# XuyangBai/D3Feat

Measured on AMD Instinct MI355X. Metric: fragments/sec (30k-pt clouds), higher is better.
Workload: dtype f32; 1 GPU; SURVEY §8d config #2: synthetic 3DMatch room fragment, 300k raw pts -> grid subsample 0.03 m (~29k pts per cloud) -> self-pair -> 5-level pyramid -> full KPFCNN forward (random-init weights (reference initialiser, seed 42), 14.1M params)...; points_per_cloud=29369, fragments_per_gpu=2141, parallelism=fragment-dp1, fragments_per_replay=12, engine_fallbacks=0, engine_isolated_replays=0

## Files before the change

### d3feat_amd/csrc/pool_head.hip

```cpp
#include "common.h"

template <int VEC, class FT = float, bool U24 = false>
__global__ void __launch_bounds__(256) maxpool_kernel(const FT* __restrict__ x, int N1, int ldx, int C,
                                                      const int* __restrict__ idx, int N2, int ld_idx, int K,
                                                      FT* __restrict__ out, int ldo,
                                                      const int* __restrict__ N1_dev, const int* __restrict__ N2_dev,
                                                      const int* __restrict__ row_order) {
    N1 = d3f_dyn(N1, N1_dev);
    N2 = d3f_dyn(N2, N2_dev);
    const int CV = C / VEC;
    const unsigned nblk = (unsigned)(((long long)N2 * CV + 255) / 256);
    if (blockIdx.x >= nblk) return;
    const long long t = (long long)d3f_xcd_tile(blockIdx.x, nblk) * 256 + threadIdx.x;
    if (t >= (long long)N2 * CV) return;
    int slot, c;
    if (U24) { const unsigned tu = (unsigned)t; slot = (int)(tu / (unsigned)CV); c = (int)(tu - (unsigned)slot * (unsigned)CV) * VEC; }
    else { slot = (int)(t / CV); c = (int)(t % CV) * VEC; }
    const int n = row_order ? row_order[slot] : slot;
    float m[VEC];
#pragma unroll
    for (int v = 0; v < VEC; ++v) m[v] = -3.402823466e38f;
    const int* row = U24 ? idx + __umul24((unsigned)n, (unsigned)ld_idx) : idx + (size_t)n * ld_idx;
    int nvalid = 0;
    constexpr int NB = 8;
    for (int k0 = 0; k0 < K; k0 += NB) {
        int id[NB];
        float val[NB][VEC];
#pragma unroll
        for (int j = 0; j < NB; ++j) id[j] = (k0 + j < K) ? row[k0 + j] : -2;
#pragma unroll
        for (int j = 0; j < NB; ++j) {
            const bool ok = id[j] >= 0 && id[j] < N1;
            nvalid += ok ? 1 : 0;
            if (ok) {
                const FT* xr = U24 ? x + (__umul24((unsigned)id[j], (unsigned)ldx) + (unsigned)c) : x + ((size_t)id[j] * ldx + c);
                if (VEC == 4) {
                    const float4 f = D3fFeat<FT>::ld4(xr);
                    val[j][0] = f.x; val[j][1 % VEC] = f.y; val[j][2 % VEC] = f.z; val[j][3 % VEC] = f.w;
                } else {
#pragma unroll
                    for (int v = 0; v < VEC; ++v) val[j][v] = D3fFeat<FT>::ld1(xr + v);
                }
            } else {
#pragma unroll
                for (int v = 0; v < VEC; ++v) val[j][v] = -3.402823466e38f;
            }
        }
#pragma unroll
        for (int j = 0; j < NB; ++j)
#pragma unroll
            for (int v = 0; v < VEC; ++v) m[v] = fmaxf(m[v], val[j][v]);
    }
    if (nvalid == 0) {
        unsigned om[VEC];
#pragma unroll
        for (int v = 0; v < VEC; ++v) om[v] = 0xFFFFFFFFu;
        for (int r0 = 0; r0 < N1; r0 += 4) {
            float val[4][VEC];
#pragma unroll
            for (int j = 0; j < 4; ++j) {
                const int r = min(r0 + j, N1 - 1);
                const FT* xr = x + ((size_t)r * ldx + c);
                if (VEC == 4) {
                    const float4 f = D3fFeat<FT>::ld4(xr);
                    val[j][0] = f.x; val[j][1 % VEC] = f.y; val[j][2 % VEC] = f.z; val[j][3 % VEC] = f.w;
                } else {
#pragma unroll
                    for (int v = 0; v < VEC; ++v) val[j][v] = D3fFeat<FT>::ld1(xr + v);
                }
            }
#pragma unroll
            for (int j = 0; j < 4; ++j)
#pragma unroll
                for (int v = 0; v < VEC; ++v) om[v] = min(om[v], d3f_f2ord(val[j][v]));
        }
#pragma unroll
        for (int v = 0; v < VEC; ++v) m[v] = d3f_ord2f(om[v]);
    }
#pragma unroll
    for (int v = 0; v < VEC; ++v) D3fFeat<FT>::st1(&out[(size_t)n * ldo + c + v], m[v]);
}

extern "C" int d3f_ind_max_pool(const void* x_, int N1, int ldx, int C, const int* idx, int N2, int ld_idx, int K,
                                void* out_, int ldo, float* col_min_dev, const int* N1_dev, const int* N2_dev,
                                const int* row_order, int feat_bf16, void* stream_) {
    hipStream_t stream = (hipStream_t)stream_;
    const float* x = (const float*)x_;
    float* out = (float*)out_;
    (void)col_min_dev;
    if (N1 < 0 || N2 < 0 || C < 1 || ldx < C || ldo < C || K < 0 || ld_idx < K) return D3F_ERR_ARG;
    if (N2 == 0) return D3F_OK;
    if (!x || !idx || !out) return D3F_ERR_ARG;
    const bool u24 = d3f_fits_u24(N1, ldx) && d3f_fits_u24(N2, ld_idx) && (long long)N2 * C < (1ll << 31);
    if (feat_bf16) {
        if (C % 4 || ldx % 4 || ((uintptr_t)x_ & 7)) return D3F_ERR_ARG;
        const unsigned short* xh = (const unsigned short*)x_;
        unsigned short* oh = (unsigned short*)out_;
        if (u24)
            maxpool_kernel<4, unsigned short, true><<<d3f_cdiv((long long)N2 * (C / 4), 256), 256, 0, stream>>>(
                xh, N1, ldx, C, idx, N2, ld_idx, K, oh, ldo, N1_dev, N2_dev, row_order);
        else
            maxpool_kernel<4, unsigned short><<<d3f_cdiv((long long)N2 * (C / 4), 256), 256, 0, stream>>>(
                xh, N1, ldx, C, idx, N2, ld_idx, K, oh, ldo, N1_dev, N2_dev, row_order);
        D3F_LAUNCH_CHECK();
        return D3F_OK;
    }
    if (C % 4 == 0 && ldx % 4 == 0 && (((uintptr_t)x) & 15) == 0 && u24)
        maxpool_kernel<4, float, true><<<d3f_cdiv((long long)N2 * (C / 4), 256), 256, 0, stream>>>(x, N1, ldx, C, idx, N2, ld_idx, K,
                                                                                                   out, ldo, N1_dev, N2_dev, row_order);
    else if (C % 4 == 0 && ldx % 4 == 0 && (((uintptr_t)x) & 15) == 0)
        maxpool_kernel<4><<<d3f_cdiv((long long)N2 * (C / 4), 256), 256, 0, stream>>>(x, N1, ldx, C, idx, N2, ld_idx, K,
                                                                                      out, ldo, N1_dev, N2_dev, row_order);
    else
        maxpool_kernel<1><<<d3f_cdiv((long long)N2 * C, 256), 256, 0, stream>>>(x, N1, ldx, C, idx, N2, ld_idx, K,
                                                                               out, ldo, N1_dev, N2_dev, row_order);
    D3F_LAUNCH_CHECK();
    return D3F_OK;
}

__global__ void __launch_bounds__(256) upsample_cat_kernel(const float* __restrict__ x, int N1, int ldx, int C1,
                                                           const int* __restrict__ idx, int N2, int ld_idx,
                                                           const float* __restrict__ skip, int lds, int C2,
                                                           float* __restrict__ out, int ldo, const int* __restrict__ N1_dev,
                                                           const int* __restrict__ N2_dev) {
    N1 = d3f_dyn(N1, N1_dev);
    N2 = d3f_dyn(N2, N2_dev);
    const int Ct = C1 + C2;
    const long long t = (long long)blockIdx.x * blockDim.x + threadIdx.x;
    if (t >= (long long)N2 * Ct) return;
    const int n = (int)(t / Ct), c = (int)(t % Ct);
    float v;
    if (c < C1) {
        const int id = idx[(size_t)n * ld_idx];
        v = (id >= 0 && id < N1) ? x[(size_t)id * ldx + c] : 0.f;
    } else {
        v = skip[(size_t)n * lds + (c - C1)];
    }
    out[(size_t)n * ldo + c] = v;
}

extern "C" int d3f_closest_pool_cat(const float* x, int N1, int ldx, int C1, const int* idx, int N2, int ld_idx,
                                    const float* skip, int lds, int C2, float* out, int ldo, const int* N1_dev,
                                    const int* N2_dev, void* stream_) {
    hipStream_t stream = (hipStream_t)stream_;
    if (N1 < 0 || N2 < 0 || C1 < 1 || C2 < 0 || ldx < C1 || ldo < C1 + C2 || ld_idx < 1 || (C2 > 0 && lds < C2))
        return D3F_ERR_ARG;
    if (N2 == 0) return D3F_OK;
    if (!x || !idx || !out || (C2 > 0 && !skip)) return D3F_ERR_ARG;
    upsample_cat_kernel<<<d3f_cdiv((long long)N2 * (C1 + C2), 256), 256, 0, stream>>>(x, N1, ldx, C1, idx, N2, ld_idx, skip,
                                                                                      lds, C2, out, ldo, N1_dev, N2_dev);
    D3F_LAUNCH_CHECK();
    return D3F_OK;
}

__global__ void __launch_bounds__(256) head_max_init_kernel(const int* __restrict__ lens, const int* __restrict__ include_zero_dev,
                                                            int group, int B, unsigned* __restrict__ mx, int* __restrict__ offs) {
    __shared__ int slen[256];
    const int b = threadIdx.x;
    const int len = b < B ? lens[b] : 0;
    const int inc_in = (include_zero_dev && b < B) ? include_zero_dev[b] : 0;
    slen[b] = len;
    __syncthreads();
    if (b >= B) return;
    const int g = group > 0 ? group : B;
    const int g0 = b / g * g, g1 = min(g0 + g, B);
    int before = 0;
    for (int j = 0; j < b; ++j) before += slen[j];
    int longest = 0, all_eq = 1;
    for (int j = g0; j < g1; ++j) longest = max(longest, slen[j]);
    for (int j = g0; j < g1; ++j) all_eq &= (slen[j] == longest);
    offs[b] = before;
    const int inc = include_zero_dev ? inc_in : ((len < longest || all_eq) ? 1 : 0);
    mx[b] = inc ? d3f_f2ord(0.f) : 0u;
    if (b == B - 1) offs[B] = before + len;
}

template <bool DENSE>
__global__ void __launch_bounds__(256) head_max_kernel(const float* __restrict__ x, int N, int ldx, int C,
                                                       const int* __restrict__ offs, int B, unsigned* __restrict__ mx) {
    const int b = blockIdx.y;
    const long long lo = (long long)offs[b] * C, hi = (long long)offs[b + 1] * C;
    unsigned m = 0u;
    if (DENSE) {
        const long long lo4 = lo >> 2, hi4 = hi >> 2;
        const long long stride = (long long)gridDim.x * blockDim.x;
        long long t = lo4 + (long long)blockIdx.x * blockDim.x + threadIdx.x;
        for (; t + 3 * stride < hi4; t += 4 * stride) {
            float4 v[4];
#pragma unroll
            for (int u = 0; u < 4; ++u) v[u] = ((const float4*)x)[t + u * stride];
#pragma unroll
            for (int u = 0; u < 4; ++u)
                m = max(max(m, d3f_f2ord(v[u].x)), max(d3f_f2ord(v[u].y), max(d3f_f2ord(v[u].z), d3f_f2ord(v[u].w))));
        }
        for (; t < hi4; t += stride) {
            const float4 v = ((const float4*)x)[t];
            m = max(max(m, d3f_f2ord(v.x)), max(d3f_f2ord(v.y), max(d3f_f2ord(v.z), d3f_f2ord(v.w))));
        }
    } else {
        for (long long t = lo + (long long)blockIdx.x * blockDim.x + threadIdx.x; t < hi; t += (long long)gridDim.x * blockDim.x) {
            const long long r = t / C;
            const int c = (int)(t % C);
            m = max(m, d3f_f2ord(x[(size_t)r * ldx + c]));
        }
    }
#pragma unroll
    for (int o = 32; o > 0; o >>= 1) m = max(m, (unsigned)__shfl_xor((int)m, o, 64));
    __shared__ unsigned red[4];
    if ((threadIdx.x & 63) == 0) red[threadIdx.x >> 6] = m;
    __syncthreads();
    if (threadIdx.x == 0 && lo < hi) atomicMax(&mx[b], max(max(red[0], red[1]), max(red[2], red[3])));
}

template <int CPL>
__global__ void __launch_bounds__(256)
head_kernel(const float* __restrict__ x, int N, int ldx, int C, const int* __restrict__ idx, int ld_idx, int K,
            const int* __restrict__ offs, int B, const unsigned* __restrict__ mx, float* __restrict__ desc, int ldd,
            float* __restrict__ score, const int* __restrict__ row_order) {
    N = min(N, offs[B]);
    if ((int)(blockIdx.x * 8) >= N) return;
    const int half = (int)d3f_xcd_tile(blockIdx.x, (unsigned)((N + 7) / 8)) * 8 + (threadIdx.x >> 5), l = threadIdx.x & 31;
    const bool active = half < N;
    const int n = active ? (row_order ? row_order[half] : half) : 0;
    const int b = d3f_find_elem(offs, B, n);
    const float den = d3f_ord2f(mx[b]) + 1e-6f;
    float xv[CPL], yv[CPL], sum[CPL];
    float sq = 0.f;
#pragma unroll
    for (int j = 0; j < CPL; ++j) {
        const int c = l + 32 * j;
        xv[j] = (c < C) ? x[(size_t)n * ldx + c] : 0.f;
        yv[j] = xv[j] / den;
        sum[j] = 0.f;
        sq += xv[j] * xv[j];
    }
#pragma unroll
    for (int o = 16; o > 0; o >>= 1) sq += __shfl_xor(sq, o, 64);
    int cnt = 0;
    const int hbase = threadIdx.x & 32;
    for (int k0 = 0; k0 < K; k0 += 32) {
        const int mine = (k0 + l < K) ? idx[(size_t)n * ld_idx + k0 + l] : -1;
        const int kn = min(32, K - k0);
        for (int kk = 0; kk < kn; kk += 4) {
            int id[4];
            float dn[4];
            float v[4][CPL];
#pragma unroll
            for (int j = 0; j < 4; ++j) {
                id[j] = __shfl(mine, hbase + min(kk + j, 31), 64);
                if (kk + j >= kn || id[j] < 0 || id[j] >= N) id[j] = -1;
            }
#pragma unroll
            for (int j = 0; j < 4; ++j) {
                dn[j] = 1.f;
                if (id[j] >= 0) dn[j] = d3f_ord2f(mx[d3f_find_elem(offs, B, id[j])]) + 1e-6f;
#pragma unroll
                for (int jj = 0; jj < CPL; ++jj) {
                    const int c = l + 32 * jj;
                    v[j][jj] = (id[j] >= 0 && c < C) ? x[(size_t)id[j] * ldx + c] : 0.f;
                }
            }
#pragma unroll
            for (int j = 0; j < 4; ++j) {
                float rs = 0.f;
#pragma unroll
                for (int jj = 0; jj < CPL; ++jj) {
                    const float y = v[j][jj] / dn[j];
                    sum[jj] += y;
                    rs += y;
                }
#pragma unroll
                for (int o = 16; o > 0; o >>= 1) rs += __shfl_xor(rs, o, 64);
                cnt += (id[j] >= 0 && rs != 0.f) ? 1 : 0;
            }
        }
    }
    const float fc = (float)max(cnt, 1);
    float ymax = -3.402823466e38f;
#pragma unroll
    for (int j = 0; j < CPL; ++j)
        if (l + 32 * j < C) ymax = fmaxf(ymax, yv[j]);
#pragma unroll
    for (int o = 16; o > 0; o >>= 1) ymax = fmaxf(ymax, __shfl_xor(ymax, o, 64));
    float best = -3.402823466e38f;
#pragma unroll
    for (int j = 0; j < CPL; ++j) {
        if (l + 32 * j < C) {
            const float d = yv[j] - sum[j] / fc;
            float sp;
            if (d > 15.f) sp = d;
            else if (d < -15.f) sp = expf(d);
            else sp = log1pf(expf(d));
            best = fmaxf(best, sp * (yv[j] / (1e-6f + ymax)));
        }
    }
#pragma unroll
    for (int o = 16; o > 0; o >>= 1) best = fmaxf(best, __shfl_xor(best, o, 64));
    if (active) {
        const float inv = rsqrtf(fmaxf(sq, 1e-10f));
#pragma unroll
        for (int j = 0; j < CPL; ++j)
            if (l + 32 * j < C) desc[(size_t)n * ldd + l + 32 * j] = xv[j] * inv;
        if (l == 0) score[n] = best;
    }
}

__global__ void __launch_bounds__(256) head32_rowflag_kernel(const float* __restrict__ x, int N, int ldx, const int* __restrict__ offs,
                                                             int B, const unsigned* __restrict__ mx, unsigned char* __restrict__ nz) {
    const int n = blockIdx.x * blockDim.x + threadIdx.x;
    if (n >= min(N, offs[B])) return;
    const int b = d3f_find_elem(offs, B, n);
    const float rden = 1.0f / (d3f_ord2f(mx[b]) + 1e-6f);
    float s[8];
#pragma unroll
    for (int j = 0; j < 8; ++j) {
        const float4 v = *(const float4*)&x[(size_t)n * ldx + 4 * j];
        s[j] = (v.x * rden + v.y * rden) + (v.z * rden + v.w * rden);
    }
    const float t0 = s[0] + s[1], t1 = s[2] + s[3], t2 = s[4] + s[5], t3 = s[6] + s[7];
    const float rs = (t0 + t1) + (t2 + t3);
    nz[n] = rs != 0.f ? 1 : 0;
}

template <bool U24>
__global__ void __launch_bounds__(256)
head32_kernel(const float* __restrict__ x, int N, int ldx, const int* __restrict__ idx, int ld_idx, int K,
              const int* __restrict__ offs, int B, const unsigned* __restrict__ mx, const unsigned char* __restrict__ nz,
              float* __restrict__ desc, int ldd, float* __restrict__ score, const int* __restrict__ row_order) {
    N = min(N, offs[B]);
    if ((int)(blockIdx.x * 8) >= N) return;
    const int half = (int)d3f_xcd_tile(blockIdx.x, (unsigned)((N + 7) / 8)) * 8 + (threadIdx.x >> 5), l = threadIdx.x & 31;
    const bool active = half < N;
    const int n = active ? (row_order ? row_order[half] : half) : 0;
    const int slot = l >> 3, c4 = (l & 7) << 2;
    const int b = d3f_find_elem(offs, B, n);
    const float den = d3f_ord2f(mx[b]) + 1e-6f;
    const float rden = 1.0f / den;
    const float4 xv = *(const float4*)&x[(size_t)n * ldx + c4];
    const float4 yv = make_float4(xv.x * rden, xv.y * rden, xv.z * rden, xv.w * rden);
    float sq = xv.x * xv.x + xv.y * xv.y + xv.z * xv.z + xv.w * xv.w;
    sq += __shfl_xor(sq, 1, 64); sq += __shfl_xor(sq, 2, 64); sq += __shfl_xor(sq, 4, 64);
    typedef float hd_f2 __attribute__((ext_vector_type(2)));
    hd_f2 sum01 = {0.f, 0.f}, sum23 = {0.f, 0.f};
    int cnt = 0;
    const int hbase = threadIdx.x & 32;
    const __amdgpu_buffer_rsrc_t xbuf = __builtin_amdgcn_make_buffer_rsrc((void*)x, 0, (int)((unsigned)N * (unsigned)ldx * 4u), 0x00020000);
    for (int k0 = 0; k0 < K; k0 += 32) {
        int mine = (k0 + l < K) ? idx[(size_t)n * ld_idx + k0 + l] : -1;
        const bool valid = mine >= 0 && mine < N;
        const bool counts = valid && nz[valid ? mine : 0] != 0;
        cnt += __popcll((__ballot(counts) >> hbase) & 0xFFFFFFFFull);
        const int kn = min(32, K - k0);
        if (U24) {
            mine = valid ? mine : N;
            for (int kk = 0; kk < kn; kk += 16) {
                float4 v[4];
#pragma unroll
                for (int u = 0; u < 4; ++u) {
                    const int idu = __shfl(mine, hbase + kk + u * 4 + slot, 64);
                    const unsigned off = (__umul24((unsigned)idu, (unsigned)ldx) + (unsigned)c4) * 4u;
                    typedef unsigned hd_u4 __attribute__((ext_vector_type(4)));
                    const hd_u4 w = __builtin_amdgcn_raw_buffer_load_b128(xbuf, (int)off, 0, 0);
                    v[u] = make_float4(__uint_as_float(w.x), __uint_as_float(w.y), __uint_as_float(w.z), __uint_as_float(w.w));
                }
                const hd_f2 r2 = {rden, rden};
#pragma unroll
                for (int u = 0; u < 4; ++u) {
                    const hd_f2 v01 = {v[u].x, v[u].y}, v23 = {v[u].z, v[u].w};
                    sum01 = sum01 + v01 * r2;
                    sum23 = sum23 + v23 * r2;
                }
            }
        } else {
            if (!valid) mine = -1;
            for (int kk = 0; kk < kn; kk += 16) {
                int id[4];
                float4 v[4];
#pragma unroll
                for (int u = 0; u < 4; ++u) {
                    const int kq = kk + u * 4 + slot;
                    id[u] = __shfl(mine, hbase + min(kq, 31), 64);
                    if (kq >= kn) id[u] = -1;
                    const float4 t = *(const float4*)(x + ((size_t)max(id[u], 0) * ldx + c4));
                    v[u] = id[u] < 0 ? make_float4(0.f, 0.f, 0.f, 0.f) : t;
                }
#pragma unroll
                for (int u = 0; u < 4; ++u) {
                    const float r = id[u] < 0 ? 0.f : rden;
                    const hd_f2 r2 = {r, r}, v01 = {v[u].x, v[u].y}, v23 = {v[u].z, v[u].w};
                    sum01 = sum01 + v01 * r2;
                    sum23 = sum23 + v23 * r2;
                }
            }
        }
    }
    float4 sum = make_float4(sum01.x, sum01.y, sum23.x, sum23.y);
    sum.x += __shfl_xor(sum.x, 8, 64); sum.y += __shfl_xor(sum.y, 8, 64); sum.z += __shfl_xor(sum.z, 8, 64); sum.w += __shfl_xor(sum.w, 8, 64);
    sum.x += __shfl_xor(sum.x, 16, 64); sum.y += __shfl_xor(sum.y, 16, 64); sum.z += __shfl_xor(sum.z, 16, 64); sum.w += __shfl_xor(sum.w, 16, 64);
    const float fc = (float)max(cnt, 1);
    float ymax = fmaxf(fmaxf(yv.x, yv.y), fmaxf(yv.z, yv.w));
    ymax = fmaxf(ymax, __shfl_xor(ymax, 1, 64)); ymax = fmaxf(ymax, __shfl_xor(ymax, 2, 64)); ymax = fmaxf(ymax, __shfl_xor(ymax, 4, 64));
    const float yj = slot == 0 ? yv.x : slot == 1 ? yv.y : slot == 2 ? yv.z : yv.w;
    const float sj = slot == 0 ? sum.x : slot == 1 ? sum.y : slot == 2 ? sum.z : sum.w;
    const float d = yj - sj / fc;
    float sp;
    if (d > 15.f) sp = d;
    else if (d < -15.f) sp = expf(d);
    else sp = log1pf(expf(d));
    float best = sp * (yj / (1e-6f + ymax));
    best = fmaxf(best, __shfl_xor(best, 1, 64)); best = fmaxf(best, __shfl_xor(best, 2, 64)); best = fmaxf(best, __shfl_xor(best, 4, 64));
    best = fmaxf(best, __shfl_xor(best, 8, 64)); best = fmaxf(best, __shfl_xor(best, 16, 64));
    if (active && slot == 0) {
        const float inv = rsqrtf(fmaxf(sq, 1e-10f));
        *(float4*)&desc[(size_t)n * ldd + c4] = make_float4(xv.x * inv, xv.y * inv, xv.z * inv, xv.w * inv);
        if (l == 0) score[n] = best;
    }
}

extern "C" int d3f_detect_head(const float* x, int N, int ldx, int C, const int* idx, int ld_idx, int K,
                               const int* lens_dev, const int* include_zero_dev, int stack_group, int B, float* desc, int ldd,
                               float* score, int* scratch_dev, const int* row_order, void* stream_) {
    hipStream_t stream = (hipStream_t)stream_;
    if (N < 0 || C < 1 || C > 128 || ldx < C || ldd < C || K < 0 || ld_idx < K || B < 1 || B > D3F_MAX_BATCH || stack_group < 0)
        return D3F_ERR_ARG;
    if (N == 0) return D3F_OK;
    if (!x || !idx || !lens_dev || !desc || !score || !scratch_dev) return D3F_ERR_ARG;
    unsigned* mx = (unsigned*)scratch_dev;
    int* offs = scratch_dev + B;
    head_max_init_kernel<<<1, 256, 0, stream>>>(lens_dev, include_zero_dev, stack_group, B, mx, offs);
    int chunks = d3f_cdiv((long long)N * C, 256 * 16);
    const int fill = d3f_cdiv(512, B);
    if (chunks > fill) chunks = fill;
    if (chunks < 1) chunks = 1;
    if (ldx == C && C % 4 == 0 && ((uintptr_t)x & 15) == 0) head_max_kernel<true><<<dim3(chunks, B), 256, 0, stream>>>(x, N, ldx, C, offs, B, mx);
    else head_max_kernel<false><<<dim3(chunks, B), 256, 0, stream>>>(x, N, ldx, C, offs, B, mx);
    const int blocks = d3f_cdiv((long long)N * 32, 256);
    const bool vec32 = C == 32 && ldx % 4 == 0 && ldd % 4 == 0 && (((uintptr_t)x | (uintptr_t)desc) & 15) == 0;
    if (vec32) {
        unsigned char* nz = (unsigned char*)(scratch_dev + 2 * B + 2);
        head32_rowflag_kernel<<<d3f_cdiv(N, 256), 256, 0, stream>>>(x, N, ldx, offs, B, mx, nz);
        if (d3f_fits_u24(N + 1, ldx) && ((long long)N + 1) * ldx < (1ll << 30))
            head32_kernel<true><<<blocks, 256, 0, stream>>>(x, N, ldx, idx, ld_idx, K, offs, B, mx, nz, desc, ldd, score, row_order);
        else
            head32_kernel<false><<<blocks, 256, 0, stream>>>(x, N, ldx, idx, ld_idx, K, offs, B, mx, nz, desc, ldd, score, row_order);
    }
    else if (C <= 32) head_kernel<1><<<blocks, 256, 0, stream>>>(x, N, ldx, C, idx, ld_idx, K, offs, B, mx, desc, ldd, score, row_order);
    else if (C <= 64) head_kernel<2><<<blocks, 256, 0, stream>>>(x, N, ldx, C, idx, ld_idx, K, offs, B, mx, desc, ldd, score, row_order);
    else head_kernel<4><<<blocks, 256, 0, stream>>>(x, N, ldx, C, idx, ld_idx, K, offs, B, mx, desc, ldd, score, row_order);
    D3F_LAUNCH_CHECK();
    return D3F_OK;
}

__global__ void __launch_bounds__(256) affine_act_kernel(const float* __restrict__ x, int ldx, int M, int N,
                                                         const float* __restrict__ cs, const float* __restrict__ ch,
                                                         const float* __restrict__ res, int ldr, int leaky, float alpha,
                                                         float* __restrict__ out, int ldo, const int* __restrict__ M_dev) {
    M = d3f_dyn(M, M_dev);
    const long long t = (long long)blockIdx.x * blockDim.x + threadIdx.x;
    if (t >= (long long)M * N) return;
    const int m = (int)(t / N), n = (int)(t % N);
    float v = x[(size_t)m * ldx + n];
    if (cs) v *= cs[n];
    if (ch) v += ch[n];
    if (res) v += res[(size_t)m * ldr + n];
    if (leaky) v = v > 0.f ? v : v * alpha;
    out[(size_t)m * ldo + n] = v;
}

extern "C" int d3f_affine_act(const float* x, int ldx, int M, int N, const float* col_scale, const float* col_shift,
                              const float* residual, int ldr, int leaky, float alpha, float* out, int ldo,
                              const int* M_dev, void* stream_) {
    hipStream_t stream = (hipStream_t)stream_;
    if (M < 0 || N < 0 || ldx < N || ldo < N || (residual && ldr < N)) return D3F_ERR_ARG;
    if (M == 0 || N == 0) return D3F_OK;
    if (!x || !out) return D3F_ERR_ARG;
    affine_act_kernel<<<d3f_cdiv((long long)M * N, 256), 256, 0, stream>>>(x, ldx, M, N, col_scale, col_shift, residual, ldr,
                                                                          leaky, alpha, out, ldo, M_dev);
    D3F_LAUNCH_CHECK();
    return D3F_OK;
}

__global__ void __launch_bounds__(256) pack_rows_kernel(const float* __restrict__ xyz, const float* __restrict__ desc, int ldd,
                                                        int C, const float* __restrict__ score, int N,
                                                        const int* __restrict__ N_dev, float* __restrict__ out, int ldo,
                                                        const int* __restrict__ lens_dev, int B, int group, int keep,
                                                        const long long* __restrict__ dst_ptrs, const int* __restrict__ row_map) {
    __shared__ int sStart[D3F_MAX_BATCH + 1];
    N = d3f_dyn(N, N_dev);
    if (dst_ptrs) {
        if (threadIdx.x == 0) {
            int s = 0;
            for (int b = 0; b < B; ++b) { sStart[b] = s; s += lens_dev[b]; }
            sStart[B] = s;
        }
        __syncthreads();
    }
    const int W = C + 4, Q = W >> 2;
    const long long t = (long long)blockIdx.x * blockDim.x + threadIdx.x;
    if (t >= (long long)N * Q) return;
    const int n = (int)(t / Q), q = (int)(t - (long long)n * Q);
    float v[4];
#pragma unroll
    for (int u = 0; u < 4; ++u) {
        const int c = 4 * q + u;
        v[u] = c < 3 ? xyz[3 * (size_t)n + c] : (c < 3 + C ? desc[(size_t)n * ldd + (c - 3)] : score[n]);
    }
    const int no = row_map ? row_map[n] : n;
    float* dst = out + (size_t)no * ldo + 4 * q;
    if (dst_ptrs) {
        int b = 0;
        while (b + 1 < B && no >= sStart[b + 1]) ++b;
        const int f = b / group;
        const long long base = dst_ptrs[f];
        if (base != 0 && b - f * group < keep) dst = (float*)base + (size_t)(no - sStart[f * group]) * ldo + 4 * q;
    }
    *(float4*)dst = make_float4(v[0], v[1], v[2], v[3]);
}

__global__ void __launch_bounds__(256) pack_rows_scalar_kernel(const float* __restrict__ xyz, const float* __restrict__ desc, int ldd,
                                                               int C, const float* __restrict__ score, int N,
                                                               const int* __restrict__ N_dev, float* __restrict__ out, int ldo) {
    N = d3f_dyn(N, N_dev);
    const int W = C + 4;
    const long long t = (long long)blockIdx.x * blockDim.x + threadIdx.x;
    if (t >= (long long)N * W) return;
    const int n = (int)(t / W), c = (int)(t % W);
    out[(size_t)n * ldo + c] = c < 3 ? xyz[3 * (size_t)n + c] : (c < 3 + C ? desc[(size_t)n * ldd + (c - 3)] : score[n]);
}

static int pack_launch(const float* xyz, const float* desc, int ldd, int C, const float* score, int N, float* out, int ldo,
                       const int* N_dev, const int* lens_dev, int B, int group, int keep, const long long* dst_ptrs, const int* row_map,
                       hipStream_t stream) {
    if (N < 0 || C < 1 || ldd < C || ldo < C + 4) return D3F_ERR_ARG;
    if (N == 0) return D3F_OK;
    if (!xyz || !desc || !score || !out) return D3F_ERR_ARG;
    if (((C + 4) & 3) || (ldo & 3) || ((uintptr_t)out & 15)) {
        if (dst_ptrs || row_map) return D3F_ERR_ARG;
        pack_rows_scalar_kernel<<<d3f_cdiv((long long)N * (C + 4), 256), 256, 0, stream>>>(xyz, desc, ldd, C, score, N, N_dev, out, ldo);
        D3F_LAUNCH_CHECK();
        return D3F_OK;
    }
    pack_rows_kernel<<<d3f_cdiv((long long)N * ((C + 4) / 4), 256), 256, 0, stream>>>(xyz, desc, ldd, C, score, N, N_dev, out, ldo, lens_dev,
                                                                                   B, group, keep, dst_ptrs, row_map);
    D3F_LAUNCH_CHECK();
    return D3F_OK;
}

extern "C" int d3f_pack_descriptors(const float* xyz, const float* desc, int ldd, int C, const float* score, int N, float* out,
                                    int ldo, const int* N_dev, void* stream_) {
    return pack_launch(xyz, desc, ldd, C, score, N, out, ldo, N_dev, nullptr, 0, 1, 0, nullptr, nullptr, (hipStream_t)stream_);
}

extern "C" int d3f_pack_descriptors_to(const float* xyz, const float* desc, int ldd, int C, const float* score, int N, float* out,
                                       int ldo, const int* N_dev, const int* lens_dev, int B, int group, int keep,
                                       const long long* dst_ptrs_dev, const int* row_map_dev, void* stream_) {
    if (dst_ptrs_dev && (!lens_dev || B < 1 || B > D3F_MAX_BATCH || group < 1 || keep < 0 || keep > group)) return D3F_ERR_ARG;
    if (!dst_ptrs_dev && !row_map_dev) return D3F_ERR_ARG;
    return pack_launch(xyz, desc, ldd, C, score, N, out, ldo, N_dev, lens_dev, B, group, keep, dst_ptrs_dev, row_map_dev,
                       (hipStream_t)stream_);
}

__device__ __forceinline__ float rec_coord(const unsigned char* __restrict__ p, int is_f64, int swap) {
    if (is_f64) {
        unsigned long long u = 0;
#pragma unroll
        for (int b = 0; b < 8; ++b) u |= (unsigned long long)p[swap ? 7 - b : b] << (8 * b);
        return (float)__longlong_as_double((long long)u);
    }
    unsigned u = 0;
#pragma unroll
    for (int b = 0; b < 4; ++b) u |= (unsigned)p[swap ? 3 - b : b] << (8 * b);
    return __uint_as_float(u);
}

__global__ void __launch_bounds__(256) decode_records_kernel(const unsigned char* __restrict__ raw, int n, int stride, int ox,
                                                             int oy, int oz, int is_f64, int swap, float* __restrict__ out) {
    const int i = blockIdx.x * blockDim.x + threadIdx.x;
    if (i >= n) return;
    const unsigned char* r = raw + (size_t)i * stride;
    out[3 * (size_t)i] = rec_coord(r + ox, is_f64, swap);
    out[3 * (size_t)i + 1] = rec_coord(r + oy, is_f64, swap);
    out[3 * (size_t)i + 2] = rec_coord(r + oz, is_f64, swap);
}

extern "C" int d3f_decode_xyz_records(const void* raw, int n, int stride, int off_x, int off_y, int off_z, int is_f64,
                                      int big_endian, float* out, void* stream_) {
    hipStream_t stream = (hipStream_t)stream_;
    const int w = is_f64 ? 8 : 4;
    if (n < 0 || stride < 3 * w || off_x < 0 || off_y < 0 || off_z < 0 || off_x + w > stride || off_y + w > stride ||
        off_z + w > stride)
        return D3F_ERR_ARG;
    if (n == 0) return D3F_OK;
    if (!raw || !out) return D3F_ERR_ARG;
    decode_records_kernel<<<d3f_cdiv(n, 256), 256, 0, stream>>>((const unsigned char*)raw, n, stride, off_x, off_y, off_z,
                                                                is_f64 ? 1 : 0, big_endian ? 1 : 0, out);
    D3F_LAUNCH_CHECK();
    return D3F_OK;
}

extern "C" int d3f_version(void) { return 200; }
```

Measured before the change: 1904 fragments/s.

## Add wave-cooperative maxpool kernel that compacts neighbor indices through LDS

Adds a maxpool kernel in which a wavefront loads a row's neighbor indices cooperatively, filters out invalid ones with ballot and popcount, and writes the compacted list to shared memory. Each lane then reads the list with vector loads and gathers D feature rows at once, so the index validity checks and per-lane index loads are not repeated in every channel lane. For C=128 the two half-waves cover different output rows. It is used for C of 128 or a multiple of 256 in both fp32 and bf16, and adds wave barriers and LDS traffic that depend on lanes within a wave sharing the same row.

```diff
diff --git a/d3feat_amd/csrc/pool_head.hip b/d3feat_amd/csrc/pool_head.hip
--- a/d3feat_amd/csrc/pool_head.hip
+++ b/d3feat_amd/csrc/pool_head.hip
@@ -81,6 +81,126 @@
     for (int v = 0; v < VEC; ++v) D3fFeat<FT>::st1(&out[(size_t)n * ldo + c + v], m[v]);
 }
 
+#define MP_LIST 80
+template <class FT, bool U24, bool HALF, int D>
+__global__ void __launch_bounds__(256) maxpool_rows_kernel(const FT* __restrict__ x, int N1, int ldx, int C,
+                                                           const int* __restrict__ idx, int N2, int ld_idx, int K,
+                                                           FT* __restrict__ out, int ldo, int ovec,
+                                                           const int* __restrict__ N1_dev, const int* __restrict__ N2_dev,
+                                                           const int* __restrict__ row_order) {
+    static_assert(D % 4 == 0 && D <= 16, "16-byte index reads inside MP_LIST");
+    __shared__ __attribute__((aligned(16))) int slist[4][HALF ? 2 : 1][MP_LIST];
+    N1 = d3f_dyn(N1, N1_dev);
+    N2 = d3f_dyn(N2, N2_dev);
+    const int CV = C >> 2;
+    const unsigned nblk = (unsigned)(((long long)N2 * CV + 255) / 256);
+    if (blockIdx.x >= nblk) return;
+    const long long t = (long long)d3f_xcd_tile(blockIdx.x, nblk) * 256 + threadIdx.x;
+    const bool live = t < (long long)N2 * CV;
+    if (!HALF && !live) return;
+    int slot = 0, c = 0;
+    if (live) {
+        if (U24) { const unsigned tu = (unsigned)t; slot = (int)(tu / (unsigned)CV); c = (int)(tu - (unsigned)slot * (unsigned)CV) * 4; }
+        else { slot = (int)(t / CV); c = (int)(t % CV) * 4; }
+    }
+    const int n = live ? (row_order ? row_order[slot] : slot) : 0;
+    const int lane = threadIdx.x & 63;
+    const int l = HALF ? (lane & 31) : lane, hs = HALF ? (lane >> 5) : 0;
+    int* lst = slist[threadIdx.x >> 6][hs];
+    const int* row = U24 ? idx + __umul24((unsigned)n, (unsigned)ld_idx) : idx + (size_t)n * ld_idx;
+    float m[4];
+#pragma unroll
+    for (int v = 0; v < 4; ++v) m[v] = -3.402823466e38f;
+    int nvalid = 0;
+    for (int k0 = 0; k0 < K; k0 += 64) {
+        int nv;
+        if (HALF) {
+            const int ka = k0 + l, kb = k0 + 32 + l;
+            const int ia = (live && ka < K) ? row[ka] : -1, ib = (live && kb < K) ? row[kb] : -1;
+            const bool va = ia >= 0 && ia < N1, vb = ib >= 0 && ib < N1;
+            const unsigned ma = (unsigned)(__ballot(va) >> (hs * 32)), mb = (unsigned)(__ballot(vb) >> (hs * 32));
+            const unsigned lt = (1u << l) - 1u;
+            const int na = __popc(ma);
+            if (va) lst[__popc(ma & lt)] = ia;
+            if (vb) lst[na + __popc(mb & lt)] = ib;
+            nv = na + __popc(mb);
+        } else {
+            const int ka = k0 + l;
+            const int ia = ka < K ? row[ka] : -1;
+            const bool va = ia >= 0 && ia < N1;
+            const unsigned long long ma = __ballot(va);
+            if (va) lst[__popcll(ma & d3f_lanemask_lt())] = ia;
+            nv = __builtin_amdgcn_readfirstlane(__popcll(ma));
+        }
+        nvalid += nv;
+        __builtin_amdgcn_fence(__ATOMIC_RELEASE, "wavefront");
+        __builtin_amdgcn_wave_barrier();
+        __builtin_amdgcn_fence(__ATOMIC_ACQUIRE, "wavefront");
+        const int nvw = HALF ? __builtin_amdgcn_readfirstlane(max(nv, __shfl_xor(nv, 32, 64))) : nv;
+        for (int j0 = 0; j0 < nvw; j0 += D) {
+            int id[D];
+            float4 val[D];
+#pragma unroll
+            for (int q = 0; q < D / 4; ++q) {
+                const int4 w = *(const int4*)(lst + j0 + 4 * q);
+                id[4 * q] = w.x; id[4 * q + 1] = w.y; id[4 * q + 2] = w.z; id[4 * q + 3] = w.w;
+            }
+#pragma unroll
+            for (int u = 0; u < D; ++u) {
+                if (j0 + u < nv) {
+                    const FT* xr = U24 ? x + (__umul24((unsigned)id[u], (unsigned)ldx) + (unsigned)c) : x + ((size_t)id[u] * ldx + c);
+                    val[u] = D3fFeat<FT>::ld4(xr);
+                } else {
+                    val[u] = make_float4(-3.402823466e38f, -3.402823466e38f, -3.402823466e38f, -3.402823466e38f);
+                }
+            }
+#pragma unroll
+            for (int u = 0; u < D; ++u) {
+                m[0] = fmaxf(m[0], val[u].x); m[1] = fmaxf(m[1], val[u].y); m[2] = fmaxf(m[2], val[u].z); m[3] = fmaxf(m[3], val[u].w);
+            }
+        }
+        __builtin_amdgcn_wave_barrier();
+    }
+    if (!live) return;
+    if (nvalid == 0) {
+        unsigned om[4];
+#pragma unroll
+        for (int v = 0; v < 4; ++v) om[v] = 0xFFFFFFFFu;
+        for (int r0 = 0; r0 < N1; r0 += 4) {
+            float4 val[4];
+#pragma unroll
+            for (int j = 0; j < 4; ++j) val[j] = D3fFeat<FT>::ld4(x + ((size_t)min(r0 + j, N1 - 1) * ldx + c));
+#pragma unroll
+            for (int j = 0; j < 4; ++j) {
+                om[0] = min(om[0], d3f_f2ord(val[j].x)); om[1] = min(om[1], d3f_f2ord(val[j].y));
+                om[2] = min(om[2], d3f_f2ord(val[j].z)); om[3] = min(om[3], d3f_f2ord(val[j].w));
+            }
+        }
+#pragma unroll
+        for (int v = 0; v < 4; ++v) m[v] = d3f_ord2f(om[v]);
+    }
+    FT* o = out + ((size_t)n * ldo + c);
+    if (ovec) D3fFeat<FT>::st4(o, make_float4(m[0], m[1], m[2], m[3]));
+    else {
+#pragma unroll
+        for (int v = 0; v < 4; ++v) D3fFeat<FT>::st1(o + v, m[v]);
+    }
+}
+
+#define MP_D (sizeof(FT) == 4 ? 16 : 8)
+template <class FT>
+static void maxpool_rows_launch(const FT* x, int N1, int ldx, int C, const int* idx, int N2, int ld_idx, int K, FT* out, int ldo,
+                                const int* N1_dev, const int* N2_dev, const int* row_order, bool u24, hipStream_t stream) {
+    const int blocks = d3f_cdiv((long long)N2 * (C / 4), 256);
+    const int ovec = (ldo % 4 == 0 && ((uintptr_t)out & (4 * sizeof(FT) - 1)) == 0) ? 1 : 0;
+#define MP_GO(U, H) maxpool_rows_kernel<FT, U, H, MP_D><<<blocks, 256, 0, stream>>>(x, N1, ldx, C, idx, N2, ld_idx, K, out, ldo, ovec, \
+                                                                                   N1_dev, N2_dev, row_order)
+    if (C == 128) { if (u24) MP_GO(true, true); else MP_GO(false, true); }
+    else { if (u24) MP_GO(true, false); else MP_GO(false, false); }
+#undef MP_GO
+}
+static inline bool maxpool_rows_shape(int C) { return C == 128 || (C >= 256 && C % 256 == 0); }
+
 extern "C" int d3f_ind_max_pool(const void* x_, int N1, int ldx, int C, const int* idx, int N2, int ld_idx, int K,
                                 void* out_, int ldo, float* col_min_dev, const int* N1_dev, const int* N2_dev,
                                 const int* row_order, int feat_bf16, void* stream_) {
@@ -96,6 +216,11 @@
         if (C % 4 || ldx % 4 || ((uintptr_t)x_ & 7)) return D3F_ERR_ARG;
         const unsigned short* xh = (const unsigned short*)x_;
         unsigned short* oh = (unsigned short*)out_;
+        if (maxpool_rows_shape(C)) {
+            maxpool_rows_launch<unsigned short>(xh, N1, ldx, C, idx, N2, ld_idx, K, oh, ldo, N1_dev, N2_dev, row_order, u24, stream);
+            D3F_LAUNCH_CHECK();
+            return D3F_OK;
+        }
         if (u24)
             maxpool_kernel<4, unsigned short, true><<<d3f_cdiv((long long)N2 * (C / 4), 256), 256, 0, stream>>>(
                 xh, N1, ldx, C, idx, N2, ld_idx, K, oh, ldo, N1_dev, N2_dev, row_order);
@@ -105,7 +230,9 @@
         D3F_LAUNCH_CHECK();
         return D3F_OK;
     }
-    if (C % 4 == 0 && ldx % 4 == 0 && (((uintptr_t)x) & 15) == 0 && u24)
+    if (maxpool_rows_shape(C) && ldx % 4 == 0 && (((uintptr_t)x) & 15) == 0)
+        maxpool_rows_launch<float>(x, N1, ldx, C, idx, N2, ld_idx, K, out, ldo, N1_dev, N2_dev, row_order, u24, stream);
+    else if (C % 4 == 0 && ldx % 4 == 0 && (((uintptr_t)x) & 15) == 0 && u24)
         maxpool_kernel<4, float, true><<<d3f_cdiv((long long)N2 * (C / 4), 256), 256, 0, stream>>>(x, N1, ldx, C, idx, N2, ld_idx, K,
                                                                                                    out, ldo, N1_dev, N2_dev, row_order);
     else if (C % 4 == 0 && ldx % 4 == 0 && (((uintptr_t)x) & 15) == 0)
```

Result: no change. 1914 fragments/s (median of 6 runs) (+0.5%).
